# cvlab-kaist/3DGAN-Inversion

Measured on AMD Instinct MI355X. Metric: inversion-steps/sec (G fwd+bwd, 512^2 FFHQ EG3D) at 1/2/4/8 GPUs; final PSNR, higher is better.
Workload: dtype f32 (modulated convs: two-piece fp16 split, 3 products, range-normalised; other GEMMs bf16x6; fp32-equivalent); 1 GPU; C2: FFHQ 512^2 single-image latent inversion step (Phase A, w + 17 noise maps per image; G.synthesis fwd+bwd, 128^2 x 96-sample rendering, stub-LPIPS feature distance + noise regulariser, Adam); images_per_gpu=1, world_size=1, generator=ffhqrebalanced512-128-shaped, 30.66 M params, random-init (synthetic weights), parallelism=1 independent images, 1 per GPU; stat all-reduce only, launch=one HIP graph replay per step

## Files before the change

### 3dgan-inversion_amd/csrc/noise_ops.hip

```cpp
#include "common.h"
#include "det.h"

namespace {

constexpr int NT = 1024;
constexpr int MAXB = 32;

struct NoiseBufs {
    float* x[MAXB];
    float* g[MAXB];
    int res[MAXB];
    int64_t ws_off[MAXB];
    int n;
};

__device__ float block_sum(float v, float* red) {
    for (int m = 32; m >= 1; m >>= 1) v += __shfl_xor(v, m);
    const int w = threadIdx.x >> 6, l = threadIdx.x & 63;
    __syncthreads();
    if (l == 0) red[w] = v;
    __syncthreads();
    float t = 0.f;
    if (threadIdx.x < NT / 64) t = red[threadIdx.x];
    if (w == 0) {
        for (int m = 8; m >= 1; m >>= 1) t += __shfl_xor(t, m);
        if (l == 0) red[16] = t;
    }
    __syncthreads();
    return red[16];
}

constexpr int BAND = 64;
constexpr int CHUNK = NT * 4;
constexpr int MAXL = 12;

__host__ __device__ inline int noise_levels(int res) { int nl = 1; for (int r = res; r > 8; r >>= 1) ++nl; return nl; }
__host__ __device__ inline int noise_band(int res) { const int b = res / 8; return b < 1 ? res : (b < BAND ? (res < BAND ? res : BAND) : b); }
__host__ __device__ inline int64_t lev_off(int res, int l) {
    int64_t o = 0;
    for (int k = 1; k < l; ++k) { const int r = res >> k; o += (int64_t)r * r; }
    return o;
}

__global__ void __launch_bounds__(NT) noise_pyramid_kernel(const NoiseBufs B, float* __restrict__ ws, float* __restrict__ sums, float* __restrict__ reg_out) {
    int blk = blockIdx.x, b = 0, band = 0;
    for (; b < B.n; ++b) {
        const int nb = B.res[b] / noise_band(B.res[b]);
        if (blk < nb) { band = blk; break; }
        blk -= nb;
    }
    if (b >= B.n) return;
    if (blockIdx.x == 0 && threadIdx.x == 0) *reg_out = 0.f;
    if (band == 0 && threadIdx.x < 2 * MAXL) sums[b * 2 * MAXL + threadIdx.x] = 0.f;
    const int res = B.res[b], nl = noise_levels(res), R = noise_band(res);
    float* scratch = ws + B.ws_off[b];
    const float* cur = B.x[b];
    int r = res, rows = R, y0 = band * R;
    for (int l = 1; l < nl; ++l) {
        const int h = r >> 1, hrows = rows >> 1, hy0 = y0 >> 1;
        float* nxt = scratch + lev_off(res, l);
        const int sh = __ffs(h) - 1;
        for (int i = threadIdx.x; i < hrows * h; i += NT) {
            const int yy = i >> sh, xx = i - (yy << sh);
            const float2 p0 = *reinterpret_cast<const float2*>(cur + (int64_t)(y0 + 2 * yy) * r + 2 * xx);
            const float2 p1 = *reinterpret_cast<const float2*>(cur + (int64_t)(y0 + 2 * yy + 1) * r + 2 * xx);
            nxt[(int64_t)(hy0 + yy) * h + xx] = ((p0.x + p0.y) + (p1.x + p1.y)) * 0.25f;
        }
        __threadfence_block();
        __syncthreads();
        cur = nxt; r = h; rows = hrows; y0 = hy0;
    }
}

__device__ __forceinline__ void moments_locate(const NoiseBufs& B, int blk, int& buf, int& lev, int& start) {
    for (buf = 0; buf < B.n; ++buf) {
        const int nl = noise_levels(B.res[buf]);
        for (lev = 0; lev < nl; ++lev) {
            const int r = B.res[buf] >> lev;
            const int nb = (r * r + CHUNK - 1) / CHUNK;
            if (blk < nb) { start = blk * CHUNK; return; }
            blk -= nb;
        }
    }
    lev = -1;
}

__global__ void __launch_bounds__(NT) noise_moments2_kernel(const NoiseBufs B, const float* __restrict__ ws, float* __restrict__ sums) {
    __shared__ float red[32];
    int b, l, start;
    moments_locate(B, blockIdx.x, b, l, start);
    if (l < 0) return;
    const int res = B.res[b], r = res >> l, n = r * r, sh = __ffs(r) - 1;
    const float* v = l == 0 ? B.x[b] : ws + B.ws_off[b] + lev_off(res, l);
    float sx = 0.f, sy = 0.f;
    float c[CHUNK / NT], lx[CHUNK / NT], uy[CHUNK / NT];
#pragma unroll
    for (int u = 0; u < CHUNK / NT; ++u) {
        const int i = min(start + threadIdx.x + u * NT, n - 1);
        const int y = i >> sh, xx = i - (y << sh);
        c[u] = v[i];
        lx[u] = v[(y << sh) + ((xx - 1) & (r - 1))];
        uy[u] = v[(((y - 1) & (r - 1)) << sh) + xx];
    }
#pragma unroll
    for (int u = 0; u < CHUNK / NT; ++u)
        if (start + threadIdx.x + u * NT < n) { sx += c[u] * lx[u]; sy += c[u] * uy[u]; }
    sx = block_sum(sx, red);
    sy = block_sum(sy, red);
    if (threadIdx.x == 0) { eg3d_acc(sums + (b * MAXL + l) * 2, sx); eg3d_acc(sums + (b * MAXL + l) * 2 + 1, sy); }
}

__global__ void __launch_bounds__(NT) noise_grad_kernel(const NoiseBufs B, const float* __restrict__ ws, const float* __restrict__ sums, float* __restrict__ reg_out,
                                                        float scale) {
    int blk = blockIdx.x, b = 0;
    for (; b < B.n; ++b) {
        const int nb = (B.res[b] * B.res[b] + CHUNK - 1) / CHUNK;
        if (blk < nb) break;
        blk -= nb;
    }
    if (b >= B.n) return;
    const int res = B.res[b], nl = noise_levels(res);
    __shared__ float cx[MAXL], cy[MAXL];
    if (threadIdx.x < 16) {
        float part = 0.f;
        if (threadIdx.x < nl) {
            const int r = res >> threadIdx.x;
            const float n = (float)(r * r);
            const float mx = sums[(b * MAXL + threadIdx.x) * 2] / n, my = sums[(b * MAXL + threadIdx.x) * 2 + 1] / n;
            const float w = 2.f / n * scale / (float)(1 << (2 * threadIdx.x));
            cx[threadIdx.x] = mx * w;
            cy[threadIdx.x] = my * w;
            part = mx * mx + my * my;
        }
        for (int m = 8; m >= 1; m >>= 1) part += __shfl_xor(part, m, 16);
        if (blk == 0 && threadIdx.x == 0) eg3d_acc(reg_out, part * scale);
    }
    float* gout = B.g[b];
    if (gout == nullptr) return;
    __syncthreads();
    const float* x0 = B.x[b];
    const float* scratch = ws + B.ws_off[b];
    const int sh0 = __ffs(res) - 1, n0 = res * res;
#pragma unroll 2
    for (int i = blk * CHUNK + threadIdx.x; i < min(n0, (blk + 1) * CHUNK); i += NT) {
        const int y = i >> sh0, xx = i - (y << sh0);
        float g = 0.f;
        const float* v = x0;
        int64_t off = 0;
        for (int l = 0; l < nl; ++l) {
            const int r = res >> l, sh = sh0 - l, yl = y >> l, xl = xx >> l;
            g += cx[l] * (v[(yl << sh) + ((xl - 1) & (r - 1))] + v[(yl << sh) + ((xl + 1) & (r - 1))]) +
                 cy[l] * (v[(((yl - 1) & (r - 1)) << sh) + xl] + v[(((yl + 1) & (r - 1)) << sh) + xl]);
            v = scratch + off;
            off += (int64_t)(r >> 1) * (r >> 1);
        }
        gout[i] = g;
    }
}

__global__ void __launch_bounds__(NT) noise_normalize_kernel(const NoiseBufs B) {
    __shared__ float red[32];
    float* x = B.x[blockIdx.x];
    const int n = B.res[blockIdx.x] * B.res[blockIdx.x];
    float s = 0.f;
    for (int i = threadIdx.x; i < n; i += NT) s += x[i];
    const float mean = block_sum(s, red) / (float)n;
    float q = 0.f;
    for (int i = threadIdx.x; i < n; i += NT) { float v = x[i] - mean; q += v * v; }
    const float inv = 1.0f / sqrtf(block_sum(q, red) / (float)n);
    for (int i = threadIdx.x; i < n; i += NT) x[i] = (x[i] - mean) * inv;
}

constexpr int NORM_CHUNK = NT * 8;

__device__ __forceinline__ bool norm_locate(const NoiseBufs& B, int blk, int& buf, int& start, int& n) {
    int b0 = 0;
    for (buf = 0; buf < B.n; ++buf) {
        n = B.res[buf] * B.res[buf];
        const int nb = (n + NORM_CHUNK - 1) / NORM_CHUNK;
        if (blk < b0 + nb) { start = (blk - b0) * NORM_CHUNK; return true; }
        b0 += nb;
    }
    return false;
}

__global__ void __launch_bounds__(NT) noise_moments_kernel(const NoiseBufs B, float* __restrict__ ws) {
    __shared__ float red[32];
    int buf, start, n;
    if (!norm_locate(B, blockIdx.x, buf, start, n)) return;
    const float* x = B.x[buf];
    float s = 0.f, q = 0.f;
    for (int i = start + threadIdx.x; i < min(n, start + NORM_CHUNK); i += NT) { const float v = x[i]; s += v; q += v * v; }
    s = block_sum(s, red);
    q = block_sum(q, red);
    if (threadIdx.x == 0) { eg3d_acc(ws + 2 * buf, s); eg3d_acc(ws + 2 * buf + 1, q); }
}

__global__ void __launch_bounds__(NT) noise_apply_norm_kernel(const NoiseBufs B, const float* __restrict__ ws) {
    int buf, start, n;
    if (!norm_locate(B, blockIdx.x, buf, start, n)) return;
    float* x = B.x[buf];
    const float mean = ws[2 * buf] / (float)n;
    const float inv = 1.0f / sqrtf(ws[2 * buf + 1] / (float)n - mean * mean);
    for (int i = start + threadIdx.x; i < min(n, start + NORM_CHUNK); i += NT) x[i] = (x[i] - mean) * inv;
}

constexpr int ADAM_CHUNK = NT * 4;

__device__ __forceinline__ bool adam_locate(const eg3d_adam_list& A, int blk, int& item, int64_t& start) {
    int b0 = 0;
    for (item = 0; item < A.n; ++item) {
        const int nb = (int)((A.items[item].n + ADAM_CHUNK - 1) / ADAM_CHUNK);
        if (blk < b0 + nb) { start = (int64_t)(blk - b0) * ADAM_CHUNK; return true; }
        b0 += nb;
    }
    return false;
}

__global__ void early_stop_flag_kernel(const float* __restrict__ value, float thr, float* __restrict__ done) {
    if (*value <= thr) *done = 1.0f;
}

__global__ void __launch_bounds__(NT) adam_step_kernel(const eg3d_adam_list A, float* __restrict__ ws) {
    __shared__ float red[32];
    const float skipv = A.skip != nullptr ? *A.skip : 0.f;
    const float t = *A.step + 1.0f;
    const float lr = *A.lr;
    if (skipv != 0.f) return;
    int item;
    int64_t start;
    if (adam_locate(A, blockIdx.x, item, start)) {
        const eg3d_adam_item& it = A.items[item];
        const float bc1 = 1.0f - powf(A.beta1, t), bc2s = sqrtf(1.0f - powf(A.beta2, t));
        const float step_size = lr / bc1;
        float s = 0.f, q = 0.f;
#pragma unroll
        for (int u = 0; u < ADAM_CHUNK / NT; ++u) {
            const int64_t i = start + threadIdx.x + u * NT;
            if (i < it.n) {
                float g = it.g ? it.g[i] : 0.f;
                if (it.g2) g += it.g2[i];
                const float m = it.m[i] + (g - it.m[i]) * (1.0f - A.beta1);
                const float v = it.v[i] * A.beta2 + (1.0f - A.beta2) * g * g;
                const float x = it.p[i] - step_size * m / (sqrtf(v) / bc2s + A.eps);
                it.m[i] = m; it.v[i] = v; it.p[i] = x;
                s += x; q += x * x;
            }
        }
        if (it.normalize) {
            s = block_sum(s, red);
            q = block_sum(q, red);
            if (threadIdx.x == 0) { eg3d_acc(ws + 2 * item, s); eg3d_acc(ws + 2 * item + 1, q); }
        }
    }
    if (A.bump_step && threadIdx.x == 0) {
        __threadfence();
        unsigned* tick = reinterpret_cast<unsigned*>(ws + 2 * A.n);
        if (atomicAdd(tick, 1u) == gridDim.x - 1) { *A.step = t; *tick = 0u; }
    }
}

__global__ void __launch_bounds__(NT) adam_apply_norm_kernel(const eg3d_adam_list A, const float* __restrict__ ws) {
    int item;
    int64_t start;
    if (A.skip != nullptr && *A.skip != 0.f) return;
    if (!adam_locate(A, blockIdx.x, item, start)) return;
    const eg3d_adam_item& it = A.items[item];
    if (!it.normalize) return;
    const float mean = ws[2 * item] / (float)it.n;
    const float inv = 1.0f / sqrtf(ws[2 * item + 1] / (float)it.n - mean * mean);
#pragma unroll
    for (int u = 0; u < ADAM_CHUNK / NT; ++u) {
        const int64_t i = start + threadIdx.x + u * NT;
        if (i < it.n) it.p[i] = (it.p[i] - mean) * inv;
    }
}

int fill(NoiseBufs& B, float* const* x, float* const* g, const int32_t* res, int nbufs) {
    if (!x || !res || nbufs < 1 || nbufs > MAXB) return EG3D_ERR_INVALID;
    B.n = nbufs;
    int64_t off = 0;
    for (int i = 0; i < nbufs; ++i) {
        if (!x[i] || res[i] < 1 || (res[i] & (res[i] - 1)) || res[i] > 4096) return EG3D_ERR_INVALID;
        B.x[i] = x[i];
        B.g[i] = g ? g[i] : nullptr;
        B.res[i] = res[i];
        B.ws_off[i] = off;
        off += (int64_t)res[i] * res[i];
    }
    return EG3D_OK;
}

}

extern "C" int64_t eg3d_noise_reg_workspace_floats(const int32_t* res, int nbufs) {
    int64_t t = 0;
    for (int i = 0; i < nbufs; ++i) t += (int64_t)res[i] * res[i];
    return t + 2 * MAXL * MAXB;
}

extern "C" int eg3d_noise_regularizer(float* const* x, float* const* grad, const int32_t* res, int nbufs, float* workspace, float* reg_out, float scale,
                                      void* stream) {
    NoiseBufs B;
    int rc = fill(B, x, grad, res, nbufs);
    if (rc) return rc;
    if (!workspace || !reg_out) return EG3D_ERR_INVALID;
    hipStream_t st = (hipStream_t)stream;
    int64_t pyr = 0;
    int nb1 = 0, nb2 = 0, nb3 = 0;
    for (int i = 0; i < nbufs; ++i) {
        pyr += (int64_t)res[i] * res[i];
        nb1 += res[i] / noise_band(res[i]);
        for (int l = 0; l < noise_levels(res[i]); ++l) nb2 += eg3d_cdiv((int64_t)(res[i] >> l) * (res[i] >> l), CHUNK);
        nb3 += eg3d_cdiv((int64_t)res[i] * res[i], CHUNK);
    }
    float* sums = workspace + pyr;
    EG3D_DET_SCOPE(det, stream); EG3D_DET_BIND(det, sums, 2 * MAXL * MAXB); EG3D_DET_BIND(det, reg_out, 1); EG3D_DET_COMMIT(det);
    hipLaunchKernelGGL(noise_pyramid_kernel, dim3(nb1), dim3(NT), 0, st, B, workspace, sums, reg_out);
    hipLaunchKernelGGL(noise_moments2_kernel, dim3(nb2), dim3(NT), 0, st, B, workspace, sums);
    EG3D_DET_FLUSH(det);
    hipLaunchKernelGGL(noise_grad_kernel, dim3(nb3), dim3(NT), 0, st, B, workspace, sums, reg_out, scale);
    EG3D_DET_END(det);
    EG3D_LAUNCH_CHECK();
    return EG3D_OK;
}

extern "C" int eg3d_noise_normalize(float* const* x, const int32_t* res, int nbufs, float* workspace, void* stream) {
    NoiseBufs B;
    int rc = fill(B, x, nullptr, res, nbufs);
    if (rc) return rc;
    if (workspace == nullptr) {
        hipLaunchKernelGGL(noise_normalize_kernel, dim3(nbufs), dim3(NT), 0, (hipStream_t)stream, B);
    } else {
        int blocks = 0;
        for (int i = 0; i < nbufs; ++i) blocks += eg3d_cdiv((int64_t)res[i] * res[i], NORM_CHUNK);
        EG3D_DET_SCOPE(det, stream); EG3D_DET_BIND(det, workspace, 2 * nbufs); EG3D_DET_COMMIT(det);
        hipLaunchKernelGGL(noise_moments_kernel, dim3(blocks), dim3(NT), 0, (hipStream_t)stream, B, workspace);
        EG3D_DET_END(det);
        hipLaunchKernelGGL(noise_apply_norm_kernel, dim3(blocks), dim3(NT), 0, (hipStream_t)stream, B, workspace);
    }
    EG3D_LAUNCH_CHECK();
    return EG3D_OK;
}

extern "C" int eg3d_adam_step(const eg3d_adam_list* list, float* workspace, void* stream) {
    if (!list || !workspace || list->n < 1 || list->n > EG3D_ADAM_ITEMS_MAX || !list->lr || !list->step) return EG3D_ERR_INVALID;
    int blocks = 0, norm = 0;
    for (int i = 0; i < list->n; ++i) {
        const eg3d_adam_item& it = list->items[i];
        if (!it.p || !it.m || !it.v || (!it.g && !it.g2) || it.n < 1 || it.n > (int64_t)1 << 30) return EG3D_ERR_INVALID;
        blocks += (int)eg3d_cdiv(it.n, ADAM_CHUNK);
        norm |= it.normalize;
    }
    EG3D_DET_SCOPE(det, stream);
    if (norm) { EG3D_DET_BIND(det, workspace, 2 * list->n); }
    EG3D_DET_COMMIT(det);
    hipLaunchKernelGGL(adam_step_kernel, dim3(blocks), dim3(NT), 0, (hipStream_t)stream, *list, workspace);
    EG3D_DET_END(det);
    if (norm) hipLaunchKernelGGL(adam_apply_norm_kernel, dim3(blocks), dim3(NT), 0, (hipStream_t)stream, *list, workspace);
    EG3D_LAUNCH_CHECK();
    return EG3D_OK;
}

extern "C" int eg3d_early_stop_flag(const float* value, float threshold, float* done, void* stream) {
    if (!value || !done) return EG3D_ERR_INVALID;
    hipLaunchKernelGGL(early_stop_flag_kernel, dim3(1), dim3(1), 0, (hipStream_t)stream, value, threshold, done);
    EG3D_LAUNCH_CHECK();
    return EG3D_OK;
}
```

### 3dgan-inversion_amd/csrc/style_affine.hip

```cpp
#include "common.h"
#include "det.h"

namespace {

constexpr int ROWS_PER_BLOCK_FWD = 4;
constexpr int ROWS_PER_BLOCK_BWD = 32;

__device__ __forceinline__ int find_layer(const eg3d_style_bank& b, int tile, const int rows_per_block, int& row0) {
    int l = 0, t0 = 0;
    for (; l < b.nlayers; ++l) {
        const int nt = (b.layers[l].C + rows_per_block - 1) / rows_per_block;
        if (tile < t0 + nt) break;
        t0 += nt;
    }
    row0 = (tile - t0) * rows_per_block;
    return l;
}

__global__ void __launch_bounds__(256) style_affine_fwd_kernel(const eg3d_style_bank b) {
    int row0;
    const int l = find_layer(b, blockIdx.x, ROWS_PER_BLOCK_FWD, row0);
    if (l >= b.nlayers) return;
    const eg3d_style_layer& ly = b.layers[l];
    const int lane = threadIdx.x & 63, j = row0 + (threadIdx.x >> 6);
    if (j >= ly.C) return;
    const float* wrow = ly.weight + (int64_t)j * b.D;
    const float bias = ly.bias ? ly.bias[j] * ly.bgain : 0.f;
    for (int n = 0; n < b.N; ++n) {
        const float* x = b.ws + ((int64_t)n * b.L + ly.wrow) * b.D;
        float acc = 0.f;
        for (int k = lane * 4; k < b.D; k += 256) {
            const float4 w = *reinterpret_cast<const float4*>(wrow + k);
            const float4 v = *reinterpret_cast<const float4*>(x + k);
            acc += v.x * (w.x * ly.wgain);
            acc += v.y * (w.y * ly.wgain);
            acc += v.z * (w.z * ly.wgain);
            acc += v.w * (w.w * ly.wgain);
        }
#pragma unroll
        for (int o = 32; o >= 1; o >>= 1) acc += __shfl_xor(acc, o);
        if (lane == 0) ly.out[(int64_t)n * ly.C + j] = (acc + bias) * ly.post;
    }
}

__global__ void __launch_bounds__(256) style_demod_fwd_kernel(const eg3d_style_bank b) {
    int blk = blockIdx.x, l = 0;
    for (; l < b.nlayers; ++l) {
        const int nb = b.layers[l].wsq ? (b.N * b.layers[l].Co + 3) / 4 : 0;
        if (blk < nb) break;
        blk -= nb;
    }
    if (l >= b.nlayers) return;
    const eg3d_style_layer& ly = b.layers[l];
    const int wid = blk * 4 + (threadIdx.x >> 6), lane = threadIdx.x & 63;
    if (wid >= b.N * ly.Co) return;
    const int n = wid / ly.Co, o = wid - n * ly.Co;
    const float* s = ly.out + (int64_t)n * ly.C;
    const float* wq = ly.wsq + (int64_t)o * ly.C;
    float acc = 0.f;
    for (int k = lane; k < ly.C; k += 64) { const float sv = s[k]; acc += sv * sv * wq[k]; }
    for (int m = 32; m >= 1; m >>= 1) acc += __shfl_xor(acc, m);
    if (lane == 0) ly.d[wid] = 1.0f / sqrtf(acc + 1e-8f);
}

__global__ void __launch_bounds__(256) style_demod_bwd_kernel(const eg3d_style_bank b) {
    __shared__ float part[4][64];
    int blk = blockIdx.x, l = 0, osplit = 1, kchunks = 1;
    for (; l < b.nlayers; ++l) {
        const eg3d_style_layer& q = b.layers[l];
        int nb = 0;
        if (q.dd != nullptr && q.wsq != nullptr) {
            osplit = max(1, min(q.Co / 16, 16));
            kchunks = (q.C + 63) / 64;
            nb = kchunks * b.N * osplit;
        }
        if (blk < nb) break;
        blk -= nb;
    }
    if (l >= b.nlayers) return;
    const eg3d_style_layer& ly = b.layers[l];
    const int kc = blk % kchunks, n = (blk / kchunks) % b.N, oz = blk / (kchunks * b.N);
    const int k = kc * 64 + (threadIdx.x & 63), sl = threadIdx.x >> 6;
    const int per = (ly.Co + osplit - 1) / osplit;
    const int o_beg = oz * per, o_end = min(ly.Co, o_beg + per);
    float acc = 0.f;
    if (k < ly.C) {
        for (int o = o_beg + sl; o < o_end; o += 4) {
            const float dv = ly.d[(int64_t)n * ly.Co + o];
            acc = fmaf(ly.dd[(int64_t)n * ly.Co + o] * dv * dv * dv, ly.wsq[(int64_t)o * ly.C + k], acc);
        }
    }
    part[sl][threadIdx.x & 63] = acc;
    __syncthreads();
    if (sl == 0 && k < ly.C) {
        const float t = part[0][threadIdx.x] + part[1][threadIdx.x] + part[2][threadIdx.x] + part[3][threadIdx.x];
        eg3d_acc(ly.dout_extra + (int64_t)n * ly.C + k, -ly.out[(int64_t)n * ly.C + k] * t);
    }
}

__global__ void __launch_bounds__(128) style_affine_bwd_kernel(const eg3d_style_bank b) {
    int row0;
    const int l = find_layer(b, blockIdx.x, ROWS_PER_BLOCK_BWD, row0);
    if (l >= b.nlayers) return;
    const eg3d_style_layer& ly = b.layers[l];
    if (ly.dout == nullptr && ly.dout_extra == nullptr) return;
    const int rows = min(ROWS_PER_BLOCK_BWD, ly.C - row0);
    __shared__ float coef[ROWS_PER_BLOCK_BWD];
    for (int n = 0; n < b.N; ++n) {
        __syncthreads();
        if (threadIdx.x < rows) {
            const int64_t j = (int64_t)n * ly.C + row0 + threadIdx.x;
            coef[threadIdx.x] = ((ly.dout ? ly.dout[j] : 0.f) + (ly.dout_extra ? ly.dout_extra[j] : 0.f)) * ly.post;
        }
        __syncthreads();
        if (b.dws == nullptr) continue;
        float* dst = b.dws + ((int64_t)n * b.L + ly.wrow) * b.D;
        for (int k = threadIdx.x * 4; k < b.D; k += 512) {
            float4 acc = make_float4(0.f, 0.f, 0.f, 0.f);
            for (int r0 = 0; r0 < rows; r0 += 8) {
                float4 w[8];
#pragma unroll
                for (int u = 0; u < 8; ++u) w[u] = *reinterpret_cast<const float4*>(ly.weight + (int64_t)(row0 + min(r0 + u, rows - 1)) * b.D + k);
#pragma unroll
                for (int u = 0; u < 8; ++u) {
                    const float c = r0 + u < rows ? coef[r0 + u] : 0.f;
                    acc.x += c * (w[u].x * ly.wgain);
                    acc.y += c * (w[u].y * ly.wgain);
                    acc.z += c * (w[u].z * ly.wgain);
                    acc.w += c * (w[u].w * ly.wgain);
                }
            }
            eg3d_acc(dst + k + 0, acc.x);
            eg3d_acc(dst + k + 1, acc.y);
            eg3d_acc(dst + k + 2, acc.z);
            eg3d_acc(dst + k + 3, acc.w);
        }
    }
}

__global__ void __launch_bounds__(128) style_affine_wgrad_kernel(const eg3d_style_bank b) {
    int row0;
    const int l = find_layer(b, blockIdx.x, ROWS_PER_BLOCK_BWD, row0);
    if (l >= b.nlayers) return;
    const eg3d_style_layer& ly = b.layers[l];
    if ((ly.dweight == nullptr && ly.dbias == nullptr) || (ly.dout == nullptr && ly.dout_extra == nullptr)) return;
    const int rows = min(ROWS_PER_BLOCK_BWD, ly.C - row0);
    auto coef = [&](int n, int r) {
        const int64_t j = (int64_t)n * ly.C + row0 + r;
        return ((ly.dout ? ly.dout[j] : 0.f) + (ly.dout_extra ? ly.dout_extra[j] : 0.f)) * ly.post;
    };
    if (ly.dbias != nullptr && threadIdx.x < rows) {
        float s = 0.f;
        for (int n = 0; n < b.N; ++n) s += coef(n, threadIdx.x);
        ly.dbias[row0 + threadIdx.x] = s * ly.bgain;
    }
    if (ly.dweight == nullptr) return;
    for (int k = threadIdx.x * 4; k < b.D; k += 512) {
        for (int r = 0; r < rows; ++r) {
            float4 acc = make_float4(0.f, 0.f, 0.f, 0.f);
            for (int n = 0; n < b.N; ++n) {
                const float4 x = *reinterpret_cast<const float4*>(b.ws + ((int64_t)n * b.L + ly.wrow) * b.D + k);
                const float c = coef(n, r) * ly.wgain;
                acc.x += c * x.x; acc.y += c * x.y; acc.z += c * x.z; acc.w += c * x.w;
            }
            *reinterpret_cast<float4*>(ly.dweight + (int64_t)(row0 + r) * b.D + k) = acc;
        }
    }
}

int check_bank(const eg3d_style_bank* pb, bool bwd) {
    if (!pb) return EG3D_ERR_INVALID;
    const eg3d_style_bank& b = *pb;
    if (b.nlayers < 1 || b.nlayers > EG3D_STYLE_BANK_MAX || b.N < 1 || b.L < 1 || b.D < 4 || (b.D & 3)) return EG3D_ERR_INVALID;
    bool wants_wgrad = false;
    for (int l = 0; l < b.nlayers && l < EG3D_STYLE_BANK_MAX; ++l) wants_wgrad |= b.layers[l].dweight != nullptr || b.layers[l].dbias != nullptr;
    if (!b.ws || (bwd && !b.dws && !wants_wgrad)) return EG3D_ERR_INVALID;
    if ((reinterpret_cast<uintptr_t>(b.ws) & 15) || (bwd && (reinterpret_cast<uintptr_t>(b.dws) & 15))) return EG3D_ERR_UNSUPPORTED;
    for (int l = 0; l < b.nlayers; ++l) {
        const eg3d_style_layer& ly = b.layers[l];
        if (!ly.weight || ly.C < 1 || ly.wrow < 0 || ly.wrow >= b.L) return EG3D_ERR_INVALID;
        if (!bwd && !ly.out) return EG3D_ERR_INVALID;
        if ((reinterpret_cast<uintptr_t>(ly.weight) & 15) || (reinterpret_cast<uintptr_t>(ly.dweight) & 15)) return EG3D_ERR_UNSUPPORTED;
    }
    return EG3D_OK;
}

int total_tiles(const eg3d_style_bank& b, int rows_per_block) {
    int t = 0;
    for (int l = 0; l < b.nlayers; ++l) t += eg3d_cdiv(b.layers[l].C, rows_per_block);
    return t;
}

}

extern "C" int eg3d_style_affine_fwd(const eg3d_style_bank* pb, void* stream) {
    if (int rc = check_bank(pb, false)) return rc;
    hipLaunchKernelGGL(style_affine_fwd_kernel, dim3(total_tiles(*pb, ROWS_PER_BLOCK_FWD)), dim3(256), 0, (hipStream_t)stream, *pb);
    int dblocks = 0;
    for (int l = 0; l < pb->nlayers; ++l) {
        const eg3d_style_layer& ly = pb->layers[l];
        if (ly.wsq != nullptr) {
            if (ly.Co < 1 || ly.d == nullptr) return EG3D_ERR_INVALID;
            dblocks += (pb->N * ly.Co + 3) / 4;
        }
    }
    if (dblocks > 0) hipLaunchKernelGGL(style_demod_fwd_kernel, dim3(dblocks), dim3(256), 0, (hipStream_t)stream, *pb);
    EG3D_LAUNCH_CHECK();
    return EG3D_OK;
}

extern "C" int eg3d_style_affine_bwd(const eg3d_style_bank* pb, void* stream) {
    if (int rc = check_bank(pb, true)) return rc;
    int dblocks = 0;
    for (int l = 0; l < pb->nlayers; ++l) {
        const eg3d_style_layer& ly = pb->layers[l];
        if (ly.dd != nullptr && ly.wsq != nullptr) {
            if (ly.Co < 1 || ly.d == nullptr || ly.dout_extra == nullptr || ly.out == nullptr) return EG3D_ERR_INVALID;
            dblocks += ((ly.C + 63) / 64) * pb->N * std::max(1, std::min(ly.Co / 16, 16));
        }
    }
    EG3D_DET_SCOPE(det, stream);
    for (int l = 0; l < pb->nlayers; ++l) {
        const eg3d_style_layer& ly = pb->layers[l];
        if (ly.dd != nullptr && ly.wsq != nullptr) { EG3D_DET_BIND(det, ly.dout_extra, (int64_t)pb->N * ly.C); }
    }
    EG3D_DET_BIND(det, pb->dws, (int64_t)pb->N * pb->L * pb->D);
    EG3D_DET_COMMIT(det);
    if (dblocks > 0) hipLaunchKernelGGL(style_demod_bwd_kernel, dim3(dblocks), dim3(256), 0, (hipStream_t)stream, *pb);
    EG3D_DET_FLUSH(det);
    if (pb->dws != nullptr) hipLaunchKernelGGL(style_affine_bwd_kernel, dim3(total_tiles(*pb, ROWS_PER_BLOCK_BWD)), dim3(128), 0, (hipStream_t)stream, *pb);
    EG3D_DET_END(det);
    bool wants_wgrad = false;
    for (int l = 0; l < pb->nlayers; ++l) wants_wgrad |= pb->layers[l].dweight != nullptr || pb->layers[l].dbias != nullptr;
    if (wants_wgrad) hipLaunchKernelGGL(style_affine_wgrad_kernel, dim3(total_tiles(*pb, ROWS_PER_BLOCK_BWD)), dim3(128), 0, (hipStream_t)stream, *pb);
    EG3D_LAUNCH_CHECK();
    return EG3D_OK;
}
```

Measured before the change: 239.6 steps/s.

## Restructure style affine/demod kernels and vectorize Adam with wave-parallel tile lookup

Replaces the serial per-layer and per-item block lookup in both files with a wave-wide prefix scan plus ballot, so each block finds its layer or item in a fixed number of steps. The Adam step and normalize kernels now handle four contiguous floats per thread with float4 loads and stores, and issue those loads before reading the skip flag. The style affine forward and demod forward kernels become multi-row GEMVs that keep weight rows in registers and reuse them across the batch. The demod and affine backward kernels move to a shared column-sum routine with larger row tiles and a shared-memory reduction, which cuts the number of atomic accumulations per output. In exchange the code is more complex, register pressure rises, and the demod backward launches fewer, larger blocks, which may reduce parallelism.

Measured after the change: 243.2 steps/s, median of 6. 1.5% higher.

```diff
diff --git a/3dgan-inversion_amd/csrc/noise_ops.hip b/3dgan-inversion_amd/csrc/noise_ops.hip
--- a/3dgan-inversion_amd/csrc/noise_ops.hip
+++ b/3dgan-inversion_amd/csrc/noise_ops.hip
@@ -207,14 +207,40 @@
 
 constexpr int ADAM_CHUNK = NT * 4;
 
+static_assert(EG3D_ADAM_ITEMS_MAX <= 64, "one lane per item");
 __device__ __forceinline__ bool adam_locate(const eg3d_adam_list& A, int blk, int& item, int64_t& start) {
-    int b0 = 0;
-    for (item = 0; item < A.n; ++item) {
-        const int nb = (int)((A.items[item].n + ADAM_CHUNK - 1) / ADAM_CHUNK);
-        if (blk < b0 + nb) { start = (int64_t)(blk - b0) * ADAM_CHUNK; return true; }
-        b0 += nb;
-    }
-    return false;
+    const int lane = threadIdx.x & 63;
+    const int nb = lane < A.n ? (int)((A.items[lane].n + ADAM_CHUNK - 1) / ADAM_CHUNK) : 0;
+    int inc = nb;
+#pragma unroll
+    for (int o = 1; o < 64; o <<= 1) { const int t = __shfl_up(inc, o); if (lane >= o) inc += t; }
+    const unsigned long long m = __ballot(lane < A.n && blk < inc);
+    if (m == 0) return false;
+    item = __ffsll(m) - 1;
+    start = (int64_t)__builtin_amdgcn_readfirstlane(blk - __shfl(inc - nb, item)) * ADAM_CHUNK;
+    return true;
+}
+
+struct Quad { float e[4]; };
+__device__ __forceinline__ Quad load_quad(const float* p, int64_t i0, int64_t n, bool vec) {
+    Quad q;
+    if (vec) { const float4 t = *reinterpret_cast<const float4*>(p + i0); q.e[0] = t.x; q.e[1] = t.y; q.e[2] = t.z; q.e[3] = t.w; }
+    else {
+#pragma unroll
+        for (int e = 0; e < 4; ++e) q.e[e] = p[i0 + e < n ? i0 + e : n - 1];
+    }
+    return q;
+}
+__device__ __forceinline__ void store_quad(float* p, int64_t i0, int64_t n, bool vec, const Quad& q) {
+    if (vec) *reinterpret_cast<float4*>(p + i0) = make_float4(q.e[0], q.e[1], q.e[2], q.e[3]);
+    else {
+#pragma unroll
+        for (int e = 0; e < 4; ++e) if (i0 + e < n) p[i0 + e] = q.e[e];
+    }
+}
+__device__ __forceinline__ bool aligned16(const void* a, const void* b2 = nullptr, const void* c = nullptr, const void* d = nullptr, const void* e = nullptr) {
+    return ((reinterpret_cast<uintptr_t>(a) | reinterpret_cast<uintptr_t>(b2) | reinterpret_cast<uintptr_t>(c) | reinterpret_cast<uintptr_t>(d) |
+             reinterpret_cast<uintptr_t>(e)) & 15) == 0;
 }
 
 __global__ void early_stop_flag_kernel(const float* __restrict__ value, float thr, float* __restrict__ done) {
@@ -223,30 +249,38 @@
 
 __global__ void __launch_bounds__(NT) adam_step_kernel(const eg3d_adam_list A, float* __restrict__ ws) {
     __shared__ float red[32];
+    int item = 0;
+    int64_t start = 0;
+    const bool mine = adam_locate(A, blockIdx.x, item, start);
+    const eg3d_adam_item& it = A.items[item];
+    const int64_t i0 = start + (int64_t)threadIdx.x * 4;
+    bool vec = false;
+    Quad g, g2, m, v, p;
+    if (mine) {
+        const float* gp = it.g ? it.g : it.m;
+        const float* g2p = it.g2 ? it.g2 : it.m;
+        vec = aligned16(it.p, it.m, it.v, gp, g2p) && i0 + 4 <= it.n;
+        g = load_quad(gp, i0, it.n, vec); g2 = load_quad(g2p, i0, it.n, vec);
+        m = load_quad(it.m, i0, it.n, vec); v = load_quad(it.v, i0, it.n, vec); p = load_quad(it.p, i0, it.n, vec);
+    }
     const float skipv = A.skip != nullptr ? *A.skip : 0.f;
     const float t = *A.step + 1.0f;
     const float lr = *A.lr;
     if (skipv != 0.f) return;
-    int item;
-    int64_t start;
-    if (adam_locate(A, blockIdx.x, item, start)) {
-        const eg3d_adam_item& it = A.items[item];
+    if (mine) {
         const float bc1 = 1.0f - powf(A.beta1, t), bc2s = sqrtf(1.0f - powf(A.beta2, t));
         const float step_size = lr / bc1;
         float s = 0.f, q = 0.f;
 #pragma unroll
-        for (int u = 0; u < ADAM_CHUNK / NT; ++u) {
-            const int64_t i = start + threadIdx.x + u * NT;
-            if (i < it.n) {
-                float g = it.g ? it.g[i] : 0.f;
-                if (it.g2) g += it.g2[i];
-                const float m = it.m[i] + (g - it.m[i]) * (1.0f - A.beta1);
-                const float v = it.v[i] * A.beta2 + (1.0f - A.beta2) * g * g;
-                const float x = it.p[i] - step_size * m / (sqrtf(v) / bc2s + A.eps);
-                it.m[i] = m; it.v[i] = v; it.p[i] = x;
-                s += x; q += x * x;
-            }
-        }
+        for (int e = 0; e < 4; ++e) {
+            float gg = it.g ? g.e[e] : 0.f;
+            if (it.g2) gg += g2.e[e];
+            m.e[e] = m.e[e] + (gg - m.e[e]) * (1.0f - A.beta1);
+            v.e[e] = v.e[e] * A.beta2 + (1.0f - A.beta2) * gg * gg;
+            p.e[e] = p.e[e] - step_size * m.e[e] / (sqrtf(v.e[e]) / bc2s + A.eps);
+            if (i0 + e < it.n) { s += p.e[e]; q += p.e[e] * p.e[e]; }
+        }
+        store_quad(it.m, i0, it.n, vec, m); store_quad(it.v, i0, it.n, vec, v); store_quad(it.p, i0, it.n, vec, p);
         if (it.normalize) {
             s = block_sum(s, red);
             q = block_sum(q, red);
@@ -261,19 +295,20 @@
 }
 
 __global__ void __launch_bounds__(NT) adam_apply_norm_kernel(const eg3d_adam_list A, const float* __restrict__ ws) {
-    int item;
-    int64_t start;
-    if (A.skip != nullptr && *A.skip != 0.f) return;
+    int item = 0;
+    int64_t start = 0;
     if (!adam_locate(A, blockIdx.x, item, start)) return;
     const eg3d_adam_item& it = A.items[item];
     if (!it.normalize) return;
+    const int64_t i0 = start + (int64_t)threadIdx.x * 4;
+    const bool vec = aligned16(it.p) && i0 + 4 <= it.n;
+    Quad p = load_quad(it.p, i0, it.n, vec);
+    if (A.skip != nullptr && *A.skip != 0.f) return;
     const float mean = ws[2 * item] / (float)it.n;
     const float inv = 1.0f / sqrtf(ws[2 * item + 1] / (float)it.n - mean * mean);
 #pragma unroll
-    for (int u = 0; u < ADAM_CHUNK / NT; ++u) {
-        const int64_t i = start + threadIdx.x + u * NT;
-        if (i < it.n) it.p[i] = (it.p[i] - mean) * inv;
-    }
+    for (int e = 0; e < 4; ++e) p.e[e] = (p.e[e] - mean) * inv;
+    store_quad(it.p, i0, it.n, vec, p);
 }
 
 int fill(NoiseBufs& B, float* const* x, float* const* g, const int32_t* res, int nbufs) {
diff --git a/3dgan-inversion_amd/csrc/style_affine.hip b/3dgan-inversion_amd/csrc/style_affine.hip
--- a/3dgan-inversion_amd/csrc/style_affine.hip
+++ b/3dgan-inversion_amd/csrc/style_affine.hip
@@ -3,148 +3,223 @@
 
 namespace {
 
-constexpr int ROWS_PER_BLOCK_FWD = 4;
-constexpr int ROWS_PER_BLOCK_BWD = 32;
-
-__device__ __forceinline__ int find_layer(const eg3d_style_bank& b, int tile, const int rows_per_block, int& row0) {
-    int l = 0, t0 = 0;
-    for (; l < b.nlayers; ++l) {
-        const int nt = (b.layers[l].C + rows_per_block - 1) / rows_per_block;
-        if (tile < t0 + nt) break;
-        t0 += nt;
-    }
-    row0 = (tile - t0) * rows_per_block;
+constexpr int GEMV_ROWS = 4, GEMV_WAVES = 4, GEMV_TILE = GEMV_ROWS * GEMV_WAVES;
+constexpr int COLS_THREADS = 512, COLS_KQ = 128, COLS_RG = COLS_THREADS / COLS_KQ;
+#ifndef EG3D_STYLE_AFFINE_BWD_TILE
+#define EG3D_STYLE_AFFINE_BWD_TILE 64
+#endif
+#ifndef EG3D_STYLE_DEMOD_BWD_TILE
+#define EG3D_STYLE_DEMOD_BWD_TILE 32
+#endif
+constexpr int AFFINE_BWD_TILE = EG3D_STYLE_AFFINE_BWD_TILE;
+constexpr int DEMOD_BWD_TILE = EG3D_STYLE_DEMOD_BWD_TILE;
+constexpr int WGRAD_ROWS = 32;
+
+static_assert(EG3D_STYLE_BANK_MAX <= 64, "one lane per layer");
+template <class Tiles>
+__device__ __forceinline__ int find_tile(const eg3d_style_bank& b, int blk, Tiles tiles, int& tile) {
+    const int lane = threadIdx.x & 63;
+    const int nt = lane < b.nlayers ? tiles(b.layers[lane]) : 0;
+    int inc = nt;
+#pragma unroll
+    for (int o = 1; o < 64; o <<= 1) { const int t = __shfl_up(inc, o); if (lane >= o) inc += t; }
+    const unsigned long long m = __ballot(lane < b.nlayers && blk < inc);
+    if (m == 0) { tile = 0; return b.nlayers; }
+    const int l = __ffsll(m) - 1;
+    tile = __builtin_amdgcn_readfirstlane(blk - __shfl(inc - nt, l));
     return l;
 }
 
-__global__ void __launch_bounds__(256) style_affine_fwd_kernel(const eg3d_style_bank b) {
+__device__ __forceinline__ int find_layer(const eg3d_style_bank& b, int blk, const int rows_per_block, int& row0) {
+    const int l = find_tile(b, blk, [&](const eg3d_style_layer& q) { return (q.C + rows_per_block - 1) / rows_per_block; }, row0);
+    row0 *= rows_per_block;
+    return l;
+}
+
+__device__ __forceinline__ float4 ld4(const float* p) { return *reinterpret_cast<const float4*>(p); }
+
+template <bool SQUARE, class Emit>
+__device__ __forceinline__ void wave_rows_dot(const float* __restrict__ M, int rows, int K, int row0, float mscale, const float* __restrict__ x, int64_t xstride,
+                                              int N, const float* __restrict__ rowc, int lane, Emit emit) {
+    const bool mine = lane < GEMV_ROWS && row0 + lane < rows;
+    const float rc = (rowc != nullptr && mine) ? rowc[row0 + lane] : 0.f;
+    const int k0 = lane * 4, k1 = 256 + lane * 4;
+    const bool in0 = k0 < K, in1 = k1 < K;
+    float4 w[GEMV_ROWS][2];
+#pragma unroll
+    for (int r = 0; r < GEMV_ROWS; ++r) {
+        const float* p = M + (int64_t)min(row0 + r, rows - 1) * K;
+        w[r][0] = ld4(p + (in0 ? k0 : 0));
+        w[r][1] = ld4(p + (in1 ? k1 : 0));
+    }
+    const float4 zero = make_float4(0.f, 0.f, 0.f, 0.f);
+    float4 v0 = in0 ? ld4(x + k0) : zero, v1 = in1 ? ld4(x + k1) : zero;
+#pragma unroll
+    for (int r = 0; r < GEMV_ROWS; ++r)
+#pragma unroll
+        for (int c = 0; c < 2; ++c) { w[r][c].x *= mscale; w[r][c].y *= mscale; w[r][c].z *= mscale; w[r][c].w *= mscale; }
+    for (int n = 0; n < N; ++n) {
+        const float* xn = x + (int64_t)n * xstride;
+        if (n > 0) { v0 = in0 ? ld4(xn + k0) : zero; v1 = in1 ? ld4(xn + k1) : zero; }
+        if (SQUARE) { v0.x *= v0.x; v0.y *= v0.y; v0.z *= v0.z; v0.w *= v0.w; v1.x *= v1.x; v1.y *= v1.y; v1.z *= v1.z; v1.w *= v1.w; }
+        float acc[GEMV_ROWS];
+#pragma unroll
+        for (int r = 0; r < GEMV_ROWS; ++r) {
+            float a = v0.x * w[r][0].x;
+            a += v0.y * w[r][0].y; a += v0.z * w[r][0].z; a += v0.w * w[r][0].w;
+            a += v1.x * w[r][1].x; a += v1.y * w[r][1].y; a += v1.z * w[r][1].z; a += v1.w * w[r][1].w;
+            acc[r] = a;
+        }
+        for (int k = 512 + lane * 4; k < K; k += 256) {
+            float4 v = ld4(xn + k);
+            if (SQUARE) { v.x *= v.x; v.y *= v.y; v.z *= v.z; v.w *= v.w; }
+#pragma unroll
+            for (int r = 0; r < GEMV_ROWS; ++r) {
+                const float4 q = ld4(M + (int64_t)min(row0 + r, rows - 1) * K + k);
+                acc[r] += v.x * (q.x * mscale); acc[r] += v.y * (q.y * mscale); acc[r] += v.z * (q.z * mscale); acc[r] += v.w * (q.w * mscale);
+            }
+        }
+#pragma unroll
+        for (int r = 0; r < GEMV_ROWS; ++r)
+#pragma unroll
+            for (int o = 32; o >= 1; o >>= 1) acc[r] += __shfl_xor(acc[r], o);
+        float mine_v = acc[0];
+#pragma unroll
+        for (int r = 1; r < GEMV_ROWS; ++r) mine_v = lane == r ? acc[r] : mine_v;
+        if (mine) emit(n, row0 + lane, mine_v, rc);
+    }
+}
+
+__global__ void __launch_bounds__(GEMV_WAVES * 64) style_affine_fwd_kernel(const eg3d_style_bank b) {
     int row0;
-    const int l = find_layer(b, blockIdx.x, ROWS_PER_BLOCK_FWD, row0);
-    if (l >= b.nlayers) return;
-    const eg3d_style_layer& ly = b.layers[l];
-    const int lane = threadIdx.x & 63, j = row0 + (threadIdx.x >> 6);
-    if (j >= ly.C) return;
-    const float* wrow = ly.weight + (int64_t)j * b.D;
-    const float bias = ly.bias ? ly.bias[j] * ly.bgain : 0.f;
+    const int l = find_layer(b, blockIdx.x, GEMV_TILE, row0);
+    if (l >= b.nlayers) return;
+    const eg3d_style_layer& ly = b.layers[l];
+    const int lane = threadIdx.x & 63;
+    row0 += (threadIdx.x >> 6) * GEMV_ROWS;
+    if (row0 >= ly.C) return;
+    wave_rows_dot<false>(ly.weight, ly.C, b.D, row0, ly.wgain, b.ws + (int64_t)ly.wrow * b.D, (int64_t)b.L * b.D, b.N, ly.bias, lane, [&](int n, int j, float dot, float bias) {
+        ly.out[(int64_t)n * ly.C + j] = (dot + bias * ly.bgain) * ly.post;
+    });
+}
+
+__global__ void __launch_bounds__(GEMV_WAVES * 64) style_demod_fwd_kernel(const eg3d_style_bank b) {
+    int blk;
+    const int l = find_tile(b, blockIdx.x, [](const eg3d_style_layer& q) { return q.wsq != nullptr ? (q.Co + GEMV_TILE - 1) / GEMV_TILE : 0; }, blk);
+    if (l >= b.nlayers) return;
+    const eg3d_style_layer& ly = b.layers[l];
+    const int lane = threadIdx.x & 63, o0 = blk * GEMV_TILE + (threadIdx.x >> 6) * GEMV_ROWS;
+    if (o0 >= ly.Co) return;
+    if ((ly.C & 3) == 0 && ((reinterpret_cast<uintptr_t>(ly.wsq) | reinterpret_cast<uintptr_t>(ly.out)) & 15) == 0) {
+        wave_rows_dot<true>(ly.wsq, ly.Co, ly.C, o0, 1.0f, ly.out, ly.C, b.N, nullptr, lane, [&](int n, int o, float dot, float) {
+            ly.d[(int64_t)n * ly.Co + o] = 1.0f / sqrtf(dot + 1e-8f);
+        });
+        return;
+    }
     for (int n = 0; n < b.N; ++n) {
-        const float* x = b.ws + ((int64_t)n * b.L + ly.wrow) * b.D;
-        float acc = 0.f;
-        for (int k = lane * 4; k < b.D; k += 256) {
-            const float4 w = *reinterpret_cast<const float4*>(wrow + k);
-            const float4 v = *reinterpret_cast<const float4*>(x + k);
-            acc += v.x * (w.x * ly.wgain);
-            acc += v.y * (w.y * ly.wgain);
-            acc += v.z * (w.z * ly.wgain);
-            acc += v.w * (w.w * ly.wgain);
-        }
-#pragma unroll
-        for (int o = 32; o >= 1; o >>= 1) acc += __shfl_xor(acc, o);
-        if (lane == 0) ly.out[(int64_t)n * ly.C + j] = (acc + bias) * ly.post;
-    }
-}
-
-__global__ void __launch_bounds__(256) style_demod_fwd_kernel(const eg3d_style_bank b) {
-    int blk = blockIdx.x, l = 0;
-    for (; l < b.nlayers; ++l) {
-        const int nb = b.layers[l].wsq ? (b.N * b.layers[l].Co + 3) / 4 : 0;
-        if (blk < nb) break;
-        blk -= nb;
-    }
-    if (l >= b.nlayers) return;
-    const eg3d_style_layer& ly = b.layers[l];
-    const int wid = blk * 4 + (threadIdx.x >> 6), lane = threadIdx.x & 63;
-    if (wid >= b.N * ly.Co) return;
-    const int n = wid / ly.Co, o = wid - n * ly.Co;
-    const float* s = ly.out + (int64_t)n * ly.C;
-    const float* wq = ly.wsq + (int64_t)o * ly.C;
-    float acc = 0.f;
-    for (int k = lane; k < ly.C; k += 64) { const float sv = s[k]; acc += sv * sv * wq[k]; }
-    for (int m = 32; m >= 1; m >>= 1) acc += __shfl_xor(acc, m);
-    if (lane == 0) ly.d[wid] = 1.0f / sqrtf(acc + 1e-8f);
-}
-
-__global__ void __launch_bounds__(256) style_demod_bwd_kernel(const eg3d_style_bank b) {
-    __shared__ float part[4][64];
-    int blk = blockIdx.x, l = 0, osplit = 1, kchunks = 1;
-    for (; l < b.nlayers; ++l) {
-        const eg3d_style_layer& q = b.layers[l];
-        int nb = 0;
-        if (q.dd != nullptr && q.wsq != nullptr) {
-            osplit = max(1, min(q.Co / 16, 16));
-            kchunks = (q.C + 63) / 64;
-            nb = kchunks * b.N * osplit;
-        }
-        if (blk < nb) break;
-        blk -= nb;
-    }
-    if (l >= b.nlayers) return;
-    const eg3d_style_layer& ly = b.layers[l];
-    const int kc = blk % kchunks, n = (blk / kchunks) % b.N, oz = blk / (kchunks * b.N);
-    const int k = kc * 64 + (threadIdx.x & 63), sl = threadIdx.x >> 6;
-    const int per = (ly.Co + osplit - 1) / osplit;
-    const int o_beg = oz * per, o_end = min(ly.Co, o_beg + per);
-    float acc = 0.f;
-    if (k < ly.C) {
-        for (int o = o_beg + sl; o < o_end; o += 4) {
-            const float dv = ly.d[(int64_t)n * ly.Co + o];
-            acc = fmaf(ly.dd[(int64_t)n * ly.Co + o] * dv * dv * dv, ly.wsq[(int64_t)o * ly.C + k], acc);
-        }
-    }
-    part[sl][threadIdx.x & 63] = acc;
-    __syncthreads();
-    if (sl == 0 && k < ly.C) {
-        const float t = part[0][threadIdx.x] + part[1][threadIdx.x] + part[2][threadIdx.x] + part[3][threadIdx.x];
-        eg3d_acc(ly.dout_extra + (int64_t)n * ly.C + k, -ly.out[(int64_t)n * ly.C + k] * t);
-    }
-}
-
-__global__ void __launch_bounds__(128) style_affine_bwd_kernel(const eg3d_style_bank b) {
+        const float* s = ly.out + (int64_t)n * ly.C;
+        for (int o = o0; o < min(o0 + GEMV_ROWS, ly.Co); ++o) {
+            const float* wq = ly.wsq + (int64_t)o * ly.C;
+            float acc = 0.f;
+            for (int k = lane; k < ly.C; k += 64) { const float sv = s[k]; acc += sv * sv * wq[k]; }
+            for (int m = 32; m >= 1; m >>= 1) acc += __shfl_xor(acc, m);
+            if (lane == 0) ly.d[(int64_t)n * ly.Co + o] = 1.0f / sqrtf(acc + 1e-8f);
+        }
+    }
+}
+
+template <int TILE, int V, class Coef, class Pre, class Emit>
+__device__ __forceinline__ void block_cols_sum(const float* __restrict__ M, int rows, int K, int row0, int N, float* coef, float* part,
+                                               Coef coef_of, Pre pre, Emit emit) {
+    constexpr int U = TILE / COLS_RG, CW = COLS_KQ * V;
+    static_assert(TILE % COLS_RG == 0 && TILE <= COLS_THREADS && CW <= COLS_THREADS, "one thread per coefficient and per column of the chunk");
+    const int tid = threadIdx.x, kq = tid & (COLS_KQ - 1), rg = tid / COLS_KQ;
+    const int nrows = min(TILE, rows - row0);
+    const bool has_coef = tid < nrows;
+    for (int kc = 0; kc < K; kc += CW) {
+        const int k = kc + kq * V;
+        const bool kin = k < K, has_col = tid < CW && kc + tid < K;
+        float w[U][V];
+#pragma unroll
+        for (int u = 0; u < U; ++u) {
+            const float* p = M + (int64_t)(row0 + min(rg * U + u, nrows - 1)) * K + (kin ? k : 0);
+            if constexpr (V == 4) { const float4 q = ld4(p); w[u][0] = q.x; w[u][1] = q.y; w[u][2] = q.z; w[u][3] = q.w; }
+            else w[u][0] = *p;
+        }
+        const int crow = row0 + min(tid, nrows - 1), ecol = min(kc + tid, K - 1);
+        float c_next = coef_of(0, crow), e_next = pre(0, ecol);
+        for (int n = 0; n < N; ++n) {
+            const float c_now = c_next, e_now = e_next;
+            __syncthreads();
+            if (tid < TILE) coef[tid] = has_coef ? c_now : 0.f;
+            __syncthreads();
+            if (n + 1 < N) {
+                c_next = coef_of(n + 1, crow);
+                e_next = pre(n + 1, ecol);
+            }
+            float acc[V];
+#pragma unroll
+            for (int v = 0; v < V; ++v) acc[v] = 0.f;
+#pragma unroll
+            for (int u = 0; u < U; ++u) {
+                const float c = coef[rg * U + u];
+#pragma unroll
+                for (int v = 0; v < V; ++v) acc[v] += c * w[u][v];
+            }
+#pragma unroll
+            for (int v = 0; v < V; ++v) part[rg * CW + kq * V + v] = acc[v];
+            __syncthreads();
+            if (has_col) {
+                float sum = part[tid];
+#pragma unroll
+                for (int g = 1; g < COLS_RG; ++g) sum += part[g * CW + tid];
+                emit(n, kc + tid, sum, e_now);
+            }
+        }
+    }
+}
+
+__global__ void __launch_bounds__(COLS_THREADS) style_demod_bwd_kernel(const eg3d_style_bank b) {
+    __shared__ float coef[DEMOD_BWD_TILE];
+    __shared__ __attribute__((aligned(16))) float part[COLS_RG * COLS_KQ * 4];
+    int blk;
+    const int l = find_tile(b, blockIdx.x, [](const eg3d_style_layer& q) {
+        return (q.dd != nullptr && q.wsq != nullptr) ? (q.Co + DEMOD_BWD_TILE - 1) / DEMOD_BWD_TILE : 0; }, blk);
+    if (l >= b.nlayers) return;
+    const eg3d_style_layer& ly = b.layers[l];
+    auto coef_of = [&](int n, int o) { const float dv = ly.d[(int64_t)n * ly.Co + o]; return ly.dd[(int64_t)n * ly.Co + o] * dv * dv * dv; };
+    auto pre = [&](int n, int k) { return ly.out[(int64_t)n * ly.C + k]; };
+    auto emit = [&](int n, int k, float t, float sv) { eg3d_acc(ly.dout_extra + (int64_t)n * ly.C + k, -sv * t); };
+    if ((ly.C & 3) == 0 && (reinterpret_cast<uintptr_t>(ly.wsq) & 15) == 0)
+        block_cols_sum<DEMOD_BWD_TILE, 4>(ly.wsq, ly.Co, ly.C, blk * DEMOD_BWD_TILE, b.N, coef, part, coef_of, pre, emit);
+    else
+        block_cols_sum<DEMOD_BWD_TILE, 1>(ly.wsq, ly.Co, ly.C, blk * DEMOD_BWD_TILE, b.N, coef, part, coef_of, pre, emit);
+}
+
+__global__ void __launch_bounds__(COLS_THREADS) style_affine_bwd_kernel(const eg3d_style_bank b) {
+    __shared__ float coef[AFFINE_BWD_TILE];
+    __shared__ __attribute__((aligned(16))) float part[COLS_RG * COLS_KQ * 4];
     int row0;
-    const int l = find_layer(b, blockIdx.x, ROWS_PER_BLOCK_BWD, row0);
+    const int l = find_layer(b, blockIdx.x, AFFINE_BWD_TILE, row0);
     if (l >= b.nlayers) return;
     const eg3d_style_layer& ly = b.layers[l];
     if (ly.dout == nullptr && ly.dout_extra == nullptr) return;
-    const int rows = min(ROWS_PER_BLOCK_BWD, ly.C - row0);
-    __shared__ float coef[ROWS_PER_BLOCK_BWD];
-    for (int n = 0; n < b.N; ++n) {
-        __syncthreads();
-        if (threadIdx.x < rows) {
-            const int64_t j = (int64_t)n * ly.C + row0 + threadIdx.x;
-            coef[threadIdx.x] = ((ly.dout ? ly.dout[j] : 0.f) + (ly.dout_extra ? ly.dout_extra[j] : 0.f)) * ly.post;
-        }
-        __syncthreads();
-        if (b.dws == nullptr) continue;
-        float* dst = b.dws + ((int64_t)n * b.L + ly.wrow) * b.D;
-        for (int k = threadIdx.x * 4; k < b.D; k += 512) {
-            float4 acc = make_float4(0.f, 0.f, 0.f, 0.f);
-            for (int r0 = 0; r0 < rows; r0 += 8) {
-                float4 w[8];
-#pragma unroll
-                for (int u = 0; u < 8; ++u) w[u] = *reinterpret_cast<const float4*>(ly.weight + (int64_t)(row0 + min(r0 + u, rows - 1)) * b.D + k);
-#pragma unroll
-                for (int u = 0; u < 8; ++u) {
-                    const float c = r0 + u < rows ? coef[r0 + u] : 0.f;
-                    acc.x += c * (w[u].x * ly.wgain);
-                    acc.y += c * (w[u].y * ly.wgain);
-                    acc.z += c * (w[u].z * ly.wgain);
-                    acc.w += c * (w[u].w * ly.wgain);
-                }
-            }
-            eg3d_acc(dst + k + 0, acc.x);
-            eg3d_acc(dst + k + 1, acc.y);
-            eg3d_acc(dst + k + 2, acc.z);
-            eg3d_acc(dst + k + 3, acc.w);
-        }
-    }
+    block_cols_sum<AFFINE_BWD_TILE, 4>(ly.weight, ly.C, b.D, row0, b.N, coef, part,
+        [&](int n, int j) {
+            const int64_t i = (int64_t)n * ly.C + j;
+            return ((ly.dout ? ly.dout[i] : 0.f) + (ly.dout_extra ? ly.dout_extra[i] : 0.f)) * ly.post * ly.wgain;
+        },
+        [](int, int) { return 0.f; },
+        [&](int n, int k, float t, float) { eg3d_acc(b.dws + ((int64_t)n * b.L + ly.wrow) * b.D + k, t); });
 }
 
 __global__ void __launch_bounds__(128) style_affine_wgrad_kernel(const eg3d_style_bank b) {
     int row0;
-    const int l = find_layer(b, blockIdx.x, ROWS_PER_BLOCK_BWD, row0);
+    const int l = find_layer(b, blockIdx.x, WGRAD_ROWS, row0);
     if (l >= b.nlayers) return;
     const eg3d_style_layer& ly = b.layers[l];
     if ((ly.dweight == nullptr && ly.dbias == nullptr) || (ly.dout == nullptr && ly.dout_extra == nullptr)) return;
-    const int rows = min(ROWS_PER_BLOCK_BWD, ly.C - row0);
+    const int rows = min(WGRAD_ROWS, ly.C - row0);
     auto coef = [&](int n, int r) {
         const int64_t j = (int64_t)n * ly.C + row0 + r;
         return ((ly.dout ? ly.dout[j] : 0.f) + (ly.dout_extra ? ly.dout_extra[j] : 0.f)) * ly.post;
@@ -195,16 +270,16 @@
 
 extern "C" int eg3d_style_affine_fwd(const eg3d_style_bank* pb, void* stream) {
     if (int rc = check_bank(pb, false)) return rc;
-    hipLaunchKernelGGL(style_affine_fwd_kernel, dim3(total_tiles(*pb, ROWS_PER_BLOCK_FWD)), dim3(256), 0, (hipStream_t)stream, *pb);
+    hipLaunchKernelGGL(style_affine_fwd_kernel, dim3(total_tiles(*pb, GEMV_TILE)), dim3(GEMV_WAVES * 64), 0, (hipStream_t)stream, *pb);
     int dblocks = 0;
     for (int l = 0; l < pb->nlayers; ++l) {
         const eg3d_style_layer& ly = pb->layers[l];
         if (ly.wsq != nullptr) {
             if (ly.Co < 1 || ly.d == nullptr) return EG3D_ERR_INVALID;
-            dblocks += (pb->N * ly.Co + 3) / 4;
-        }
-    }
-    if (dblocks > 0) hipLaunchKernelGGL(style_demod_fwd_kernel, dim3(dblocks), dim3(256), 0, (hipStream_t)stream, *pb);
+            dblocks += eg3d_cdiv(ly.Co, GEMV_TILE);
+        }
+    }
+    if (dblocks > 0) hipLaunchKernelGGL(style_demod_fwd_kernel, dim3(dblocks), dim3(GEMV_WAVES * 64), 0, (hipStream_t)stream, *pb);
     EG3D_LAUNCH_CHECK();
     return EG3D_OK;
 }
@@ -216,7 +291,7 @@
         const eg3d_style_layer& ly = pb->layers[l];
         if (ly.dd != nullptr && ly.wsq != nullptr) {
             if (ly.Co < 1 || ly.d == nullptr || ly.dout_extra == nullptr || ly.out == nullptr) return EG3D_ERR_INVALID;
-            dblocks += ((ly.C + 63) / 64) * pb->N * std::max(1, std::min(ly.Co / 16, 16));
+            dblocks += eg3d_cdiv(ly.Co, DEMOD_BWD_TILE);
         }
     }
     EG3D_DET_SCOPE(det, stream);
@@ -226,13 +301,13 @@
     }
     EG3D_DET_BIND(det, pb->dws, (int64_t)pb->N * pb->L * pb->D);
     EG3D_DET_COMMIT(det);
-    if (dblocks > 0) hipLaunchKernelGGL(style_demod_bwd_kernel, dim3(dblocks), dim3(256), 0, (hipStream_t)stream, *pb);
+    if (dblocks > 0) hipLaunchKernelGGL(style_demod_bwd_kernel, dim3(dblocks), dim3(COLS_THREADS), 0, (hipStream_t)stream, *pb);
     EG3D_DET_FLUSH(det);
-    if (pb->dws != nullptr) hipLaunchKernelGGL(style_affine_bwd_kernel, dim3(total_tiles(*pb, ROWS_PER_BLOCK_BWD)), dim3(128), 0, (hipStream_t)stream, *pb);
+    if (pb->dws != nullptr) hipLaunchKernelGGL(style_affine_bwd_kernel, dim3(total_tiles(*pb, AFFINE_BWD_TILE)), dim3(COLS_THREADS), 0, (hipStream_t)stream, *pb);
     EG3D_DET_END(det);
     bool wants_wgrad = false;
     for (int l = 0; l < pb->nlayers; ++l) wants_wgrad |= pb->layers[l].dweight != nullptr || pb->layers[l].dbias != nullptr;
-    if (wants_wgrad) hipLaunchKernelGGL(style_affine_wgrad_kernel, dim3(total_tiles(*pb, ROWS_PER_BLOCK_BWD)), dim3(128), 0, (hipStream_t)stream, *pb);
+    if (wants_wgrad) hipLaunchKernelGGL(style_affine_wgrad_kernel, dim3(total_tiles(*pb, WGRAD_ROWS)), dim3(128), 0, (hipStream_t)stream, *pb);
     EG3D_LAUNCH_CHECK();
     return EG3D_OK;
 }
```
